# 0411tony/Yue

Hardware: AMD Instinct MI355X
Metric: BPR triplet-updates/sec at k=128 (S-round semantics, user rows sequential; the reference's exact sequential semantics: secondary.exact) (higher is better)
Workload: dtype f32

## Files before the change

yue_amd/csrc/bpr_host.hip:

```cpp
#include "host_common.hpp"

#include "train_kernels.hpp"
#include "round_kernels.hpp"

using yue_host::fail;
using yue_host::kr_of;
static_assert(yue::kNllSlots == yue_host::kNllSlotsHost && yue::kHeaderSlack == yue_host::kHeaderSlackHost, "host_common.hpp mirrors these");

namespace {

yue::TrainArgs make_args(yue_ctx *c, double lr, double regU, double regI) {
    yue::TrainArgs a{};
    a.P = c->P.p; a.Q = c->Q.p; a.dP = c->dP.p; a.dQ = c->dQ.p;
    a.stage = c->Q.p ? c->Q.p + (size_t)c->n * c->k : nullptr;
    a.ev_u = c->ev_u.p; a.ev_i = c->ev_i.p; a.ev_j = c->ev_j.p;
    a.indptr = c->indptr.p; a.indices = c->indices.p;
    a.nll_slots = c->scal.p;
    a.m = c->m; a.n = c->n; a.k = c->k;
    a.lr = lr;
    a.ru = (float)(lr * regU);
    a.ri = (float)(lr * regI);
    a.neg_lo = 0; a.neg_range = (int32_t)c->n;
    return a;
}
// ... 254 lines not shown
            c->Q.release();
            c->Q = bigger;
            a.Q = c->Q.p;
        }
        if (!meta) {
            HIPCHK(c->tab0.resize((size_t)c->n * yue::kStageMax));
            HIPCHK(c->tab1.resize((size_t)c->n * yue::kStageMax));
        }
        a.stage = c->Q.p + (size_t)c->n * c->k;
    }
    std::vector<int64_t> ne;
    for (int64_t r = 0; r < R; ++r) if (bounds[(size_t)r + 1] > bounds[(size_t)r]) ne.push_back(r);
    int rc;
    if (meta) {
        if (!ne.empty() && (rc = launch_round_meta(c, a, bounds))) return rc;
    } else if (!ne.empty()) {
        const int64_t r0 = ne[0];
        if ((rc = launch_round(c, a, 0, 0, bounds[(size_t)r0], bounds[(size_t)r0 + 1], 1, apply_p))) return rc;
    }
    const bool timed = c->timing_stride > 0 && !ne.empty();
    if (timed) {
        if (c->ev_used == c->ev_pool.size()) {
            hipEvent_t s, t;
            HIPCHK(hipEventCreate(&s));
            HIPCHK(hipEventCreate(&t));
            c->ev_pool.emplace_back(s, t);
            c->ev_triplets.push_back(0);
            c->ev_launches.push_back(0);
        }
        HIPCHK(hipEventRecord(c->ev_pool[c->ev_used].first, c->stream));
    }
    size_t pos = 0;
    for (int64_t r = 0; r < R; ++r) {
        if (pos < ne.size() && ne[pos] == r) {
            const int64_t e0 = bounds[(size_t)r], e1 = bounds[(size_t)r + 1];
            int64_t n0 = 0, n1 = 0;
            if (pos + 1 < ne.size()) { n0 = bounds[(size_t)ne[pos + 1]]; n1 = bounds[(size_t)ne[pos + 1] + 1]; }
            const bool seq_user = meta && user_blocks && !c->bigq;
            if ((rc = seq_user ? launch_round_u(c, a, (*user_blocks)[(size_t)r], (*user_blocks)[(size_t)r + 1], e0, e1, r)
                      : meta ? launch_round_m(c, a, e0, e1, r) : launch_round(c, a, e0, e1, n0, n1, (int)(pos & 1), apply_p))) return rc;
            ++pos;
        }
        if ((rc = after_round(r))) return rc;
    }
    if (timed) {
        HIPCHK(hipEventRecord(c->ev_pool[c->ev_used].second, c->stream));
        c->ev_triplets[c->ev_used] = bounds.back() - bounds.front();
        c->ev_launches[c->ev_used] = (int64_t)ne.size();
        c->ev_used++;
    }
    return YUE_OK;
}

void reset_round_state(yue_ctx *c) {
    (void)hipStreamSynchronize(c->stream);
    if (c->cnt0.p) (void)hipMemsetAsync(c->cnt0.p, 0, c->cnt0.n * sizeof(unsigned long long), c->stream);
    if (c->cnt1.p) (void)hipMemsetAsync(c->cnt1.p, 0, c->cnt1.n * sizeof(unsigned long long), c->stream);
    if (c->cntp0.p) (void)hipMemsetAsync(c->cntp0.p, 0, c->cntp0.n * sizeof(uint32_t), c->stream);
    if (c->cntp1.p) (void)hipMemsetAsync(c->cntp1.p, 0, c->cntp1.n * sizeof(uint32_t), c->stream);
    if (c->dP.p) (void)hipMemsetAsync(c->dP.p, 0, c->dP.n * sizeof(float), c->stream);
    if (c->dQ.p) (void)hipMemsetAsync(c->dQ.p, 0, c->dQ.n * sizeof(float), c->stream);
    (void)hipStreamSynchronize(c->stream);
}


}

namespace yue_host {
int zero_scalars(yue_ctx *c) {
    HIPCHK(hipMemsetAsync(c->scal.p, 0, (yue::kNllSlots + 8) * sizeof(double), c->stream));
    return YUE_OK;
}

int read_scalars(yue_ctx *c, double *nll, double *sp, double *sq) {
    double *sc = c->scal.p + yue::kNllSlots;
    hipLaunchKernelGGL(yue::k_sum_slots, dim3(1), dim3(64), 0, c->stream, c->scal.p, yue::kNllSlots, sc);
    double h[3];
    HIPCHK(hipMemcpyAsync(h, sc, sizeof h, hipMemcpyDeviceToHost, c->stream));
    HIPCHK(hipStreamSynchronize(c->stream));
    if (nll) *nll = h[0];
    if (sp) *sp = h[1];
    if (sq) *sq = h[2];
    return YUE_OK;
}

int sumsq_async(yue_ctx *c, const double *p_slots) {
    double *sc = c->scal.p + yue::kNllSlots;
    HIPCHK(hipMemsetAsync(sc + 1, 0, 2 * sizeof(double), c->stream));
    if (p_slots) hipLaunchKernelGGL(yue::k_sum_slots, dim3(1), dim3(64), 0, c->stream, p_slots, yue::kNllSlots, sc + 1);
    else hipLaunchKernelGGL(yue::k_sumsq, dim3(2048), dim3(256), 0, c->stream, c->P.p, c->m * c->k, sc + 1);
    hipLaunchKernelGGL(yue::k_sumsq, dim3(2048), dim3(256), 0, c->stream, c->Q.p, c->n * c->k, sc + 2);
    return YUE_OK;
}

int upload_triplets(yue_ctx *c, const int32_t *u, const int32_t *i, const int32_t *j, int64_t T, bool validate) {
    for (int64_t t = 0; validate && t < T; ++t) {
        if (u[t] < 0 || u[t] >= c->m || i[t] < 0 || i[t] >= c->n || j[t] >= c->n)
            return fail(YUE_ERR_ARG, "triplet " + std::to_string(t) + " out of range");
    }
    HIPCHK(c->xu.resize((size_t)T + yue::kHeaderSlack)); HIPCHK(c->xi.resize((size_t)T + yue::kHeaderSlack)); HIPCHK(c->xj.resize((size_t)T + yue::kHeaderSlack));
    HIPCHK(hipMemcpyAsync(c->xu.p, u, T * sizeof(int32_t), hipMemcpyHostToDevice, c->stream));
    HIPCHK(hipMemcpyAsync(c->xi.p, i, T * sizeof(int32_t), hipMemcpyHostToDevice, c->stream));
    HIPCHK(hipMemcpyAsync(c->xj.p, j, T * sizeof(int32_t), hipMemcpyHostToDevice, c->stream));
    return YUE_OK;
}
}
// ... 106 lines not shown
    }
    HIPCHK(hipGetLastError());
    HIPCHK(hipMemcpyAsync(loss_out, c->x_loss.p, T * sizeof(double), hipMemcpyDeviceToHost, c->stream));
    HIPCHK(hipStreamSynchronize(c->stream));
    return YUE_OK;
}

int yue_adam_reset(yue_ctx *c) {
    if (!c || !c->have_factors) return fail(YUE_ERR_ARG, "yue_adam_reset: no factors uploaded");
    HIPCHK(hipSetDevice(c->device));
    const size_t mk = (size_t)c->m * c->k, nk = (size_t)c->n * c->k;
    HIPCHK(c->aU_m.resize(mk)); HIPCHK(c->aU_v.resize(mk)); HIPCHK(c->aV_m.resize(nk)); HIPCHK(c->aV_v.resize(nk));
    HIPCHK(hipMemsetAsync(c->aU_m.p, 0, mk * sizeof(float), c->stream)); HIPCHK(hipMemsetAsync(c->aU_v.p, 0, mk * sizeof(float), c->stream));
    HIPCHK(hipMemsetAsync(c->aV_m.p, 0, nk * sizeof(float), c->stream)); HIPCHK(hipMemsetAsync(c->aV_v.p, 0, nk * sizeof(float), c->stream));
    HIPCHK(hipMemsetAsync(c->dP.p, 0, mk * sizeof(float), c->stream)); HIPCHK(hipMemsetAsync(c->dQ.p, 0, nk * sizeof(float), c->stream));
    c->adam_m = c->m; c->adam_n = c->n; c->adam_k = c->k;
    return YUE_OK;
}

int yue_adam_step(yue_ctx *c, const int32_t *u, const int32_t *i, const int32_t *j, int64_t T, double lr, double reg, int64_t step, double *loss_out) {
    if (!c || !c->have_factors) return fail(YUE_ERR_ARG, "yue_adam_step: no factors uploaded");
    if (T <= 0 || !u || !i || !j || step < 1) return fail(YUE_ERR_ARG, "yue_adam_step: bad argument (T > 0, step >= 1)");
    HIPCHK(hipSetDevice(c->device));
    if (c->adam_m != c->m || c->adam_n != c->n || c->adam_k != c->k) { const int rc0 = yue_adam_reset(c); if (rc0) return rc0; }
    for (int64_t t = 0; t < T; ++t)
        if (u[t] < 0 || u[t] >= c->m || i[t] < 0 || i[t] >= c->n || j[t] < 0 || j[t] >= c->n) return fail(YUE_ERR_ARG, "yue_adam_step: triplet " + std::to_string(t) + " out of range");
    int rc = upload_triplets(c, u, i, j, T, true);
    if (rc) return rc;
    if ((rc = zero_scalars(c))) return rc;
    yue::MbArgs a{};
    a.U = c->P.p; a.V = c->Q.p; a.gU = c->dP.p; a.gV = c->dQ.p; a.k = c->k; a.u = c->xu.p; a.i = c->xi.p; a.j = c->xj.p; a.T = T;
    a.reg = (float)reg; a.loss_slots = c->scal.p;
    const dim3 grid((unsigned)(((T + 31) / 32 + 3) / 4));
    switch (kr_of(c->k)) {
        case 1: hipLaunchKernelGGL(yue::k_mb_grad<1>, grid, dim3(256), 0, c->stream, a); break;
        case 2: hipLaunchKernelGGL(yue::k_mb_grad<2>, grid, dim3(256), 0, c->stream, a); break;
        default: hipLaunchKernelGGL(yue::k_mb_grad<4>, grid, dim3(256), 0, c->stream, a); break;
    }
    const double b1 = 0.9, b2 = 0.999;
    const float lr_t = (float)(lr * std::sqrt(1.0 - std::pow(b2, (double)step)) / (1.0 - std::pow(b1, (double)step)));
    const int64_t mk = c->m * (int64_t)c->k, nk = c->n * (int64_t)c->k;
    hipLaunchKernelGGL(yue::k_adam, dim3((unsigned)std::min<int64_t>(8192, (mk + 255) / 256)), dim3(256), 0, c->stream, c->P.p, c->aU_m.p, c->aU_v.p, c->dP.p, mk, lr_t, 0.9f, 0.999f, 1e-8f);
    hipLaunchKernelGGL(yue::k_adam, dim3((unsigned)std::min<int64_t>(8192, (nk + 255) / 256)), dim3(256), 0, c->stream, c->Q.p, c->aV_m.p, c->aV_v.p, c->dQ.p, nk, lr_t, 0.9f, 0.999f, 1e-8f);
    HIPCHK(hipGetLastError());
    return read_scalars(c, loss_out, nullptr, nullptr);
}

int yue_sample_negatives(yue_ctx *c, uint64_t seed, uint32_t epoch, int32_t *j_out) {
    if (!c || !c->have_inter || !j_out) return fail(YUE_ERR_ARG, "yue_sample_negatives: no interactions uploaded");
    HIPCHK(hipSetDevice(c->device));
    yue::TrainArgs a = make_args(c, 0, 0, 0);
    a.seed = seed; a.epoch = epoch;
    if (c->E > 0) {
        hipLaunchKernelGGL(yue::k_sample, dim3((unsigned)((c->E + 255) / 256)), dim3(256), 0, c->stream, a, c->E);
        HIPCHK(hipGetLastError());
        HIPCHK(hipMemcpyAsync(j_out, c->ev_j.p, c->E * sizeof(int32_t), hipMemcpyDeviceToHost, c->stream));
    }
    HIPCHK(hipStreamSynchronize(c->stream));
    return YUE_OK;
}

int yue_sumsq(yue_ctx *c, double *sp, double *sq) {
    if (!c || !c->have_factors) return fail(YUE_ERR_ARG, "yue_sumsq: no factors uploaded");
    HIPCHK(hipSetDevice(c->device));
    int rc = sumsq_async(c);
    if (rc) return rc;
    double h[2];
    HIPCHK(hipMemcpyAsync(h, c->scal.p + yue::kNllSlots + 1, sizeof h, hipMemcpyDeviceToHost, c->stream));
    HIPCHK(hipStreamSynchronize(c->stream));
    if (sp) *sp = h[0];
    if (sq) *sq = h[1];
    return YUE_OK;
}

int yue_bpr_epoch(yue_ctx *c, uint64_t seed, uint32_t epoch, int64_t round_events, double lr, double regU, double regI,
                  double *nll_out, double *sumsqP_out, double *sumsqQ_out) {
    if (!c || !c->have_factors || !c->have_inter) return fail(YUE_ERR_ARG, "yue_bpr_epoch: upload factors and interactions first");
    if (round_events < 0) return fail(YUE_ERR_ARG, "yue_bpr_epoch: round_events must be positive (or 0 for the device's default)");
    HIPCHK(hipSetDevice(c->device));
    yue::TrainArgs a = make_args(c, lr, regU, regI);
    a.seed = seed + 0x632BE59BD9B4E019ull * (uint64_t)c->rank;
    a.epoch = epoch;
    int rc = zero_scalars(c);
    if (rc) return rc;
    const int64_t E = c->E;
    if (E > 0) hipLaunchKernelGGL(yue::k_sample, dim3((unsigned)((E + 255) / 256)), dim3(256), 0, c->stream, a, E);
    if (c->opt_epoch_exact) {
        if (yue_host::on_communicator(c) && c->nranks > 1) return fail(YUE_ERR_ARG, "yue_bpr_epoch: option epoch_exact runs on one GPU (the sequential order spans all item shards)");
        if ((rc = yue_host::chain_epoch(c, lr, regU, regI))) return rc;
        if ((rc = sumsq_async(c))) return rc;
        return read_scalars(c, nll_out, sumsqP_out, sumsqQ_out);
    }
    std::vector<int64_t> bounds;
    double tot[2] = {(double)E, (double)c->n};
    if (yue_host::on_communicator(c)) {
        if ((rc = yue_allreduce_f64(c, tot, 2))) return rc;
        if ((rc = zero_scalars(c))) return rc;
    }
    const double etot = tot[0];
    if (round_events == 0 && (rc = default_round_events(c, tot[1] / c->nranks, &round_events))) return rc;
    int64_t ub = 1, group = 1;
    if ((rc = yue_epoch_plan(c->m, c->k, round_events, etot, c->nranks, &ub, &group, nullptr))) return rc;
    if (!yue_host::on_communicator(c)) group = std::max<int64_t>(1, (c->m + ub - 1) / ub);
    else group = std::max<int64_t>(1, ((int64_t)c->opt_comm_group_mb << 20) / std::max<int64_t>(1, ub * c->k * 4));
    std::vector<int64_t> ublock;
    for (int64_t u0 = 0; u0 < c->m; u0 += ub) { ublock.push_back(u0); bounds.push_back(c->h_ev_ptr[(size_t)u0]); }
    ublock.push_back(c->m); bounds.push_back(E);
    const int64_t R = (int64_t)ublock.size() - 1;
    const bool seq_user = !yue_host::on_communicator(c) && c->opt_round_user_seq && meta_path_fits(c);
    if (seq_user) {
        HIPCHK(c->d_ev_ptr.resize((size_t)c->m + 1));
        if (!c->d_ev_ptr_valid) {
            HIPCHK(hipMemcpyAsync(c->d_ev_ptr.p, c->h_ev_ptr.data(), ((size_t)c->m + 1) * sizeof(int64_t), hipMemcpyHostToDevice, c->stream));
            c->d_ev_ptr_valid = true;
        }
        HIPCHK(c->margins.resize((size_t)std::max<int64_t>(E, 1)));
    }
    c->psq_in_rounds = seq_user && c->all_users_have_events && E > 0;
    if (c->psq_in_rounds) {
        HIPCHK(c->psq_slots.resize((size_t)yue::kNllSlots));
        HIPCHK(hipMemsetAsync(c->psq_slots.p, 0, (size_t)yue::kNllSlots * sizeof(double), c->stream));
    }
    c->last_round_user_seq = 0;
    auto after = [&](int64_t r) -> int {
        if (seq_user && !c->bigq) { c->last_round_user_seq = 1; return YUE_OK; }
        if ((r + 1) % group != 0 && r + 1 != R) return YUE_OK;
        const int64_t g_first = ublock[(size_t)(r - (r % group))], g_last = ublock[(size_t)r + 1];
        const int64_t first = g_first * c->k, count = (g_last - g_first) * c->k;
        const dim3 grid((unsigned)std::min<int64_t>(4096, (count + 255) / 256));
        if (!yue_host::on_communicator(c)) {
            hipLaunchKernelGGL(yue::k_apply_range, grid, dim3(256), 0, c->stream, c->P.p, c->dP.p, first, count);
            return YUE_OK;
        }
        HIPCHK(hipEventRecord(c->ev_rounds, c->stream));
        HIPCHK(hipStreamWaitEvent(c->comm_stream, c->ev_rounds, 0));
        c->comm_collectives += 1;
        c->comm_bytes += (double)count * sizeof(float);
        if (const int rcr = yue_host::reduce_user_block(c, first, count, c->comm_stream)) return rcr;
        hipLaunchKernelGGL(yue::k_apply_range, grid, dim3(256), 0, c->comm_stream, c->P.p, c->dP.p, first, count);
        return YUE_OK;
    };
    c->comm_collectives = 0; c->comm_bytes = 0.0; c->comm_wait_ms = 0.0;
    if ((rc = run_rounds(c, a, bounds, 0, after, meta_path_fits(c), seq_user ? &ublock : nullptr))) { reset_round_state(c); return rc; }
    if (c->last_round_user_seq && E > 0)
        hipLaunchKernelGGL(yue::k_loss_margins, dim3(2048), dim3(256), 0, c->stream, c->margins.p, c->ev_j.p, E, c->scal.p);
    const bool psq_done = c->psq_in_rounds && c->last_round_user_seq;
    c->psq_in_rounds = false;
    if (yue_host::on_communicator(c)) {
        HIPCHK(hipEventRecord(c->ev_t_rounds, c->stream));
        HIPCHK(hipEventRecord(c->ev_t_comm, c->comm_stream));
    }
    HIPCHK(hipEventRecord(c->ev_comm, c->comm_stream));
    HIPCHK(hipStreamWaitEvent(c->stream, c->ev_comm, 0));
    c->comm_compute_waits = 1;
    HIPCHK(hipGetLastError());
    if ((rc = sumsq_async(c, psq_done ? c->psq_slots.p : nullptr))) return rc;
    if ((rc = read_scalars(c, nll_out, sumsqP_out, sumsqQ_out))) return rc;
    if (yue_host::on_communicator(c)) {
        float ms = 0.f;
        HIPCHK(hipEventSynchronize(c->ev_t_comm));
        HIPCHK(hipEventElapsedTime(&ms, c->ev_t_rounds, c->ev_t_comm));
        c->comm_wait_ms = ms > 0.f ? ms : 0.0;
    }
    return YUE_OK;
}

int yue_epoch_plan(int64_t m, int k, int64_t round_events, double events_total, int nranks,
                   int64_t *user_block, int64_t *blocks_per_group, int64_t *n_blocks) {
    if (m <= 0 || k <= 0 || round_events <= 0 || nranks < 1 || !(events_total >= 0.0)) return fail(YUE_ERR_ARG, "yue_epoch_plan: bad argument");
    const double per_user = events_total / (double)nranks / (double)m;
    const int64_t ub = std::max<int64_t>(1, (int64_t)std::floor((double)round_events / std::max(per_user, 1e-9) + 0.5));
    if (user_block) *user_block = ub;
    if (blocks_per_group) *blocks_per_group = std::max<int64_t>(1, (8ll << 20) / std::max<int64_t>(1, ub * k * 4));
    if (n_blocks) *n_blocks = (m + ub - 1) / ub;
    return YUE_OK;
}

int yue_default_round_events(yue_ctx *c, int64_t *out) {
    if (!c || !c->have_factors || !out) return fail(YUE_ERR_ARG, "yue_default_round_events: upload factors first (the value depends on k)");
    HIPCHK(hipSetDevice(c->device));
    double n_rows = (double)c->n;
    if (yue_host::on_communicator(c)) {
        const int rc = yue_allreduce_f64(c, &n_rows, 1);
        if (rc) return rc;
        n_rows /= c->nranks;
    }
    return default_round_events(c, n_rows, out);
}

int yue_set_kernel_timing(yue_ctx *c, int stride) {
    if (!c || stride < 0) return fail(YUE_ERR_ARG, "yue_set_kernel_timing: bad argument");
    c->timing_stride = stride;
    c->ev_used = 0;
    return YUE_OK;
}

int yue_get_kernel_timing(yue_ctx *c, double *total_ms, int64_t *launches, int64_t *triplets) {
    if (!c) return fail(YUE_ERR_ARG, "null context");
    HIPCHK(hipSetDevice(c->device));
    HIPCHK(hipStreamSynchronize(c->stream));
    double tot = 0.0;
    int64_t trip = 0, nl = 0;
    for (size_t t = 0; t < c->ev_used; ++t) {
        float ms = 0.f;
        HIPCHK(hipEventElapsedTime(&ms, c->ev_pool[t].first, c->ev_pool[t].second));
        tot += ms;
        trip += c->ev_triplets[t];
        nl += c->ev_launches[t];
    }
    if (total_ms) *total_ms = tot;
// ... 153 lines not shown
```

yue_amd/csrc/round_kernels.hpp:

```cpp
#pragma once
#include "train_kernels.hpp"

#ifdef YUE_ABL_NO_HOT
#define YUE_M_HOT(val, rs, vo, so) asm volatile("" :: "v"(val))
#else
#define YUE_M_HOT(val, rs, vo, so) YUE_BATOMIC(val, rs, vo, so)
#endif
#ifdef YUE_ABL_NO_DP
#define YUE_M_DP(val, rs, vo, so) asm volatile("" :: "v"(val))
#else
#define YUE_M_DP(val, rs, vo, so) YUE_BATOMIC(val, rs, vo, so)
#endif

#define YUE_BLOAD_NT(rs, vo, so) __builtin_bit_cast(float, __builtin_amdgcn_raw_buffer_load_b32((rs), (vo), (so), 2))
#if defined(YUE_EXP_LOAD_CACHED)
#define YUE_M_LOAD_J(rs, vo, so) YUE_BLOAD(rs, vo, so)
#define YUE_M_LOAD_I(rs, vo, so) YUE_BLOAD(rs, vo, so)
#elif defined(YUE_EXP_LOAD_NT)
#define YUE_M_LOAD_J(rs, vo, so) YUE_BLOAD_NT(rs, vo, so)
#define YUE_M_LOAD_I(rs, vo, so) YUE_BLOAD_NT(rs, vo, so)
#else
#define YUE_M_LOAD_J(rs, vo, so) YUE_BLOAD_NT(rs, vo, so)
#define YUE_M_LOAD_I(rs, vo, so) YUE_BLOAD(rs, vo, so)
#endif

#define YUE_FOLD_LD(p) __builtin_nontemporal_load(p)
#define YUE_FOLD_LDROW(p) (*(p))

namespace yue {

constexpr uint32_t kMetaStageMax = 64u;
constexpr uint32_t kMetaStageDefault = 4u;
constexpr uint32_t kMetaUnique = 1u, kMetaStaged = 2u, kMetaHot = 3u;
constexpr uint32_t kMetaFirst = 1u << 31;
constexpr int kMetaUnroll = 8;
__host__ __device__ inline uint32_t meta_kind(uint32_t w) { return w & 3u; }
__host__ __device__ inline uint32_t meta_slot(uint32_t w) { return (w >> 2) & 0x1fffffffu; }
__host__ __device__ inline bool meta_first(uint32_t w) { return (w & kMetaFirst) != 0u; }
__host__ __device__ inline uint32_t fold_count(uint32_t w) { return w >> 25; }
__host__ __device__ inline uint32_t fold_block(uint32_t w) { return w & 0x1ffffffu; }
constexpr uint32_t kLdsStaged = 1u << 31, kLdsTicket = 1u << 25;
static_assert(kMetaStageMax <= 64u, "tickets of a block must fit bits 25..30 of the LDS word");
__device__ inline uint32_t meta_of_staged(uint32_t lds) {
    const uint32_t ticket = (lds >> 25) & 63u;
    return kMetaStaged | (((lds & 0x1ffffffu) + ticket) << 2) | (ticket == 0u ? kMetaFirst : 0u);
}

struct MetaArgs {
    const int32_t *ev_i, *ev_j;
    const int64_t *bounds;
    int64_t R;
    int32_t n;
    int32_t range;
    int32_t G;
    int32_t chunk;
    uint32_t stage_max;
    uint32_t *meta_i, *meta_j;
    unsigned long long *round_rows;
    uint2 *fold;
    const uint2 *bk_touch;
    const uint32_t *bk_ptr;
};

__host__ __device__ inline int64_t fold_base(int64_t e0, int64_t r) { return (e0 + 4 * r + 3) & ~(int64_t)3; }

template <bool BUCKETED>
__global__ void __launch_bounds__(1024) k_round_meta(MetaArgs a) {
    extern __shared__ uint32_t slots[];
    __shared__ unsigned long long wsum[16];
    __shared__ unsigned long long range_base;
    const int tid = threadIdx.x, lane = tid & 63, wv = tid >> 6;
    const int64_t xcd = blockIdx.x & 7, local = blockIdx.x >> 3, per_xcd = gridDim.x >> 3;
    const int64_t rounds_here = (a.R - xcd + 7) >> 3;
    for (int64_t sq = local; sq < rounds_here * a.G; sq += per_xcd) {
        const int64_t r = (sq / a.G) * 8 + xcd;
        const int32_t g = (int32_t)(sq % a.G);
        const int32_t lo = g * a.range;
        const int32_t width = min(a.range, a.n - lo);
        const int64_t e0 = a.bounds[r], e1 = a.bounds[r + 1];
        for (int s = tid; s < a.range; s += 1024) slots[s] = 0u;
        __syncthreads();
        const uint2 *mine_t = nullptr;
        uint32_t mine_n = 0u;
        if (BUCKETED) {
            const uint32_t *bp = a.bk_ptr + r * (a.G + 1) + g;
            mine_t = a.bk_touch + 2 * e0 + bp[0];
            mine_n = bp[1] - bp[0];
        }
        if (BUCKETED) {
            for (uint32_t t = tid; t < mine_n; t += 1024) atomicAdd(&slots[mine_t[t].x - (uint32_t)lo], 1u);
        } else {
        for (int64_t eb = e0 + tid; eb < e1; eb += 1024 * kMetaUnroll) {
            int32_t vi[kMetaUnroll], vj[kMetaUnroll];
#pragma unroll
            for (int q = 0; q < kMetaUnroll; ++q) {
                const int64_t e = eb + 1024 * q;
                vj[q] = e < e1 ? a.ev_j[e] : -1; vi[q] = e < e1 ? a.ev_i[e] : 0;
            }
#pragma unroll
            for (int q = 0; q < kMetaUnroll; ++q)
                if (vj[q] >= 0) {
                    const uint32_t si = (uint32_t)(vi[q] - lo), sj = (uint32_t)(vj[q] - lo);
                    if (si < (uint32_t)width) atomicAdd(&slots[si], 1u);
                    if (sj < (uint32_t)width) atomicAdd(&slots[sj], 1u);
                }
        }
        }
        __syncthreads();
        const int s0 = tid * a.chunk;
        unsigned long long mine = 0ull;
        for (int q = 0; q < a.chunk; ++q) {
            const int s = s0 + q;
            if (s < width) { const uint32_t c = slots[s]; if (c >= 2u) mine += (1ull << 32) + (c <= a.stage_max ? c : 0u); }
        }
        unsigned long long incl = mine;
#pragma unroll
        for (int off = 1; off < 64; off <<= 1) { const unsigned long long up = __shfl_up(incl, off); if (lane >= off) incl += up; }
        if (lane == 63) wsum[wv] = incl;
        __syncthreads();
        if (tid == 0) {
            unsigned long long total = 0ull;
            for (int q = 0; q < 16; ++q) total += wsum[q];
            range_base = total ? atomicAdd(a.round_rows + r, total) : 0ull;
        }
        __syncthreads();
        unsigned long long run = range_base + incl - mine;
        for (int q = 0; q < wv; ++q) run += wsum[q];
        uint2 *fold = a.fold + fold_base(e0, r);
        for (int q = 0; q < a.chunk; ++q) {
            const int s = s0 + q;
            if (s < width) {
                const uint32_t c = slots[s];
                if (c >= 2u) {
                    const bool st = c <= a.stage_max;
                    slots[s] = st ? (kLdsStaged | ((uint32_t)run & 0x1ffffffu)) : kMetaHot;
                    fold[run >> 32] = make_uint2((uint32_t)(lo + s), st ? ((c << 25) | ((uint32_t)run & 0x1ffffffu)) : 0u);
                    run += (1ull << 32) + (st ? c : 0u);
                }
            }
        }
        __syncthreads();
        if (BUCKETED) {
            for (uint32_t t = tid; t < mine_n; t += 1024) {
                const uint2 tc = mine_t[t];
                const uint32_t sl = tc.x - (uint32_t)lo;
                const uint32_t wd = slots[sl];
                const uint32_t mw = (wd & kLdsStaged) ? meta_of_staged(atomicAdd(&slots[sl], kLdsTicket)) : wd;
                ((tc.y & 1u) ? a.meta_j : a.meta_i)[e0 + (tc.y >> 1)] = mw;
            }
        } else
        for (int64_t eb = e0 + tid; eb < e1; eb += 1024 * kMetaUnroll) {
            int32_t vi[kMetaUnroll], vj[kMetaUnroll];
#pragma unroll
            for (int q = 0; q < kMetaUnroll; ++q) {
                const int64_t e = eb + 1024 * q;
                vj[q] = e < e1 ? a.ev_j[e] : -1; vi[q] = e < e1 ? a.ev_i[e] : 0;
            }
#pragma unroll
            for (int q = 0; q < kMetaUnroll; ++q) {
                const int64_t e = eb + 1024 * q;
                if (vj[q] >= 0) {
                    const uint32_t si = (uint32_t)(vi[q] - lo), sj = (uint32_t)(vj[q] - lo);
                    if (si < (uint32_t)width) {
                        const uint32_t wd = slots[si];
                        a.meta_i[e] = (wd & kLdsStaged) ? meta_of_staged(atomicAdd(&slots[si], kLdsTicket)) : wd;
                    }
                    if (sj < (uint32_t)width) {
                        const uint32_t wd = slots[sj];
                        a.meta_j[e] = (wd & kLdsStaged) ? meta_of_staged(atomicAdd(&slots[sj], kLdsTicket)) : wd;
                    }
                } else if (g == 0 && e < e1) {
                    a.meta_i[e] = 0u; a.meta_j[e] = 0u;
                }
            }
        }
        __syncthreads();
    }
}

constexpr int kBucketShift = 15;
constexpr int kBucketRangesMax = 256;
struct BucketArgs {
    const int32_t *ev_i, *ev_j;
    const int64_t *bounds;
    int64_t R;
    int32_t G;
    uint2 *bk_touch;
    uint32_t *bk_ptr;
    uint32_t *meta_i, *meta_j;
};

__global__ void __launch_bounds__(1024) k_round_bucket(BucketArgs a) {
    __shared__ uint32_t cnt[kBucketRangesMax], off[kBucketRangesMax + 1];
    const int tid = threadIdx.x;
    for (int64_t r = blockIdx.x; r < a.R; r += gridDim.x) {
        const int64_t e0 = a.bounds[r], e1 = a.bounds[r + 1];
        for (int g = tid; g < a.G; g += 1024) cnt[g] = 0u;
        __syncthreads();
        for (int64_t eb = e0 + tid; eb < e1; eb += 1024 * kMetaUnroll) {
            int32_t vi[kMetaUnroll], vj[kMetaUnroll];
#pragma unroll
            for (int q = 0; q < kMetaUnroll; ++q) {
                const int64_t e = eb + 1024 * q;
                vj[q] = e < e1 ? a.ev_j[e] : 0; vi[q] = e < e1 ? a.ev_i[e] : -1;
            }
#pragma unroll
            for (int q = 0; q < kMetaUnroll; ++q) {
                if (vi[q] < 0) continue;
                if (vj[q] >= 0) { atomicAdd(&cnt[vi[q] >> kBucketShift], 1u); atomicAdd(&cnt[vj[q] >> kBucketShift], 1u); }
                else { a.meta_i[eb + 1024 * q] = 0u; a.meta_j[eb + 1024 * q] = 0u; }
            }
        }
        __syncthreads();
        if (tid == 0) {
            uint32_t run = 0u;
            for (int g = 0; g < a.G; ++g) { off[g] = run; run += cnt[g]; cnt[g] = 0u; }
            off[a.G] = run;
        }
        __syncthreads();
        for (int g = tid; g <= a.G; g += 1024) a.bk_ptr[r * (a.G + 1) + g] = off[g];
        uint2 *dst = a.bk_touch + 2 * e0;
        for (int64_t eb = e0 + tid; eb < e1; eb += 1024 * kMetaUnroll) {
            int32_t vi[kMetaUnroll], vj[kMetaUnroll];
#pragma unroll
            for (int q = 0; q < kMetaUnroll; ++q) {
                const int64_t e = eb + 1024 * q;
                vj[q] = e < e1 ? a.ev_j[e] : -1; vi[q] = e < e1 ? a.ev_i[e] : 0;
// ... 243 lines not shown
            for (int r = 0; r < KR; ++r) { const float a1 = p[r] * qi[r]; ai = ai + a1; const float a2 = p[r] * qj[r]; aj = aj + a2; }
            const float x = wave_sum(ai) - wave_sum(aj);
            const float c = FAST ? chain_coef_fast(x, lrf) : (float)(a.lr * (1.0 - chain_sigmoid(x)));
            xs = (unsigned)lane == t ? x : xs;
            const unsigned cli = meta_kind(mi), clj = meta_kind(mj);
            const bool uniq_i = cli == kMetaUnique, uniq_j = clj == kMetaUnique;
            const bool full_i = uniq_i || meta_first(mi), full_j = uniq_j || meta_first(mj);
            const unsigned oi = (unsigned)ti * row_bytes, oj = (unsigned)tj * row_bytes;
            const unsigned wi = uniq_i ? oi : stage0 + meta_slot(mi) * row_bytes;
            const unsigned wj = uniq_j ? oj : stage0 + meta_slot(mj) * row_bytes;
            Elem o[KR];
#pragma unroll
            for (int r = 0; r < KR; ++r) { o[r] = bpr_elem(p[r], qi[r], qj[r], c, a.ru, a.ri); p[r] = o[r].p2; }
            if (cli != kMetaHot) {
#pragma unroll
                for (int r = 0; r < KR; ++r) YUE_BSTORE(full_i ? o[r].qi2 : o[r].qi2 - qi[r], rsQ, vo[r], wi);
            } else {
#pragma unroll
                for (int r = 0; r < KR; ++r) YUE_M_HOT(o[r].qi2 - qi[r], rsdQ, vo[r], oi);
            }
            if (clj != kMetaHot) {
#pragma unroll
                for (int r = 0; r < KR; ++r) YUE_BSTORE(full_j ? o[r].qj2 : o[r].qj2 - qj[r], rsQ, vo[r], wj);
            } else {
#pragma unroll
                for (int r = 0; r < KR; ++r) YUE_M_HOT(o[r].qj2 - qj[r], rsdQ, vo[r], oj);
            }
        };
        constexpr int D = KR == 1 ? 8 : 4;
        float qi[D][KR], qj[D][KR];
#pragma unroll
        for (int s_ = 0; s_ < D; ++s_) gather(qi[s_], qj[s_], (unsigned)s_);
        for (unsigned t = 0; t < seg_len; t += D) {
#pragma unroll
            for (int s_ = 0; s_ < D; ++s_) {
                step(qi[s_], qj[s_], t + s_);
                gather(qi[s_], qj[s_], (t + s_ + D) & 63u);
            }
        }
        if ((unsigned)lane < seg_len) ra.margins[e0 + seg + lane] = xs;
    }
#pragma unroll
    for (int r = 0; r < KR; ++r) { const unsigned e = 64u * r + lane; if (e < k) prow[e] = p[r]; }
    if (ra.psq_slots) {
        double s = 0.0;
#pragma unroll
        for (int r = 0; r < KR; ++r) { const unsigned e = 64u * r + lane; const float sq = p[r] * p[r]; if (e < k) s += (double)sq; }
#pragma unroll
        for (int off = 1; off < 64; off <<= 1) s += __shfl_xor(s, off);
        if (lane == 0) atomicAdd(ra.psq_slots + (u & (kNllSlots - 1)), s);
    }
}

__global__ void __launch_bounds__(256) k_loss_margins(const float *__restrict__ x, const int32_t *__restrict__ evj, int64_t E, double *nll_slots) {
    double nl = 0.0;
    const int64_t stride = (int64_t)gridDim.x * blockDim.x;
    for (int64_t e = (int64_t)blockIdx.x * blockDim.x + threadIdx.x; e < E; e += stride)
        if (evj[e] >= 0) nl += -log(chain_sigmoid(x[e]));
#pragma unroll
    for (int off = 1; off < 64; off <<= 1) nl += __shfl_xor(nl, off);
    if ((threadIdx.x & 63) == 0 && nl != 0.0) atomicAdd(nll_slots + ((blockIdx.x * 4 + (threadIdx.x >> 6)) & (kNllSlots - 1)), nl);
}

struct FoldArgs {
    const uint2 *fold;
    const unsigned long long *round_rows;
    float *Q, *dQ;
    const float *stage;
    int k;
    uint32_t capacity;
};

template <int KR, int EPG>
__device__ __forceinline__ void fold_group(const FoldArgs &f, int lane, unsigned k, uint32_t nact, const uint2 (&ent)[4]) {
    float st[EPG][4][KR];
    unsigned el[KR];
    bool big = false;
#pragma unroll
    for (int r = 0; r < KR; ++r) el[r] = min(64u * r + lane, k - 1u);
#pragma unroll
    for (int sl = 0; sl < EPG; ++sl) {
        if ((uint32_t)sl >= nact) continue;
        const uint32_t c = fold_count(ent[sl].y);
        const bool hot = c == 0u;
        const float *src = hot ? f.dQ + (uint64_t)ent[sl].x * k : f.stage + (uint64_t)fold_block(ent[sl].y) * k;
#pragma unroll
        for (int r = 0; r < KR; ++r) st[sl][0][r] = YUE_FOLD_LD(src + el[r]);
        if (hot) {
            const float *row = f.Q + (uint64_t)ent[sl].x * k;
#pragma unroll
            for (int r = 0; r < KR; ++r) st[sl][1][r] = YUE_FOLD_LDROW(row + el[r]);
        } else {
#pragma unroll
            for (int r = 0; r < KR; ++r) st[sl][1][r] = YUE_FOLD_LD(src + (uint64_t)k + el[r]);
        }
        if (c > 2u) {
#pragma unroll
            for (unsigned q = 2; q < 4; ++q)
#pragma unroll
                for (int r = 0; r < KR; ++r) st[sl][q][r] = YUE_FOLD_LD(src + (uint64_t)(q < c ? q : 0u) * k + el[r]);
        }
        big = big || c > 4u;
    }
#pragma unroll
    for (int sl = 0; sl < EPG; ++sl) {
        if ((uint32_t)sl >= nact) continue;
        const uint32_t c = fold_count(ent[sl].y);
        const bool hot = c == 0u;
        float *row = f.Q + (uint64_t)ent[sl].x * k;
        float *dr = f.dQ + (uint64_t)ent[sl].x * k;
#pragma unroll
        for (int r = 0; r < KR; ++r) {
            const unsigned e = 64u * r + lane;
            float acc = st[sl][1][r];
// ... 72 lines not shown
```

yue_amd/csrc/train_kernels.hpp:

```cpp
#pragma once
#include "bpr_device.hpp"

namespace yue {

__global__ void __launch_bounds__(256) k_sample(TrainArgs a, int64_t E) {
    int64_t e = (int64_t)blockIdx.x * blockDim.x + threadIdx.x;
    if (e < E) a.ev_j[e] = sample_negative(a, a.ev_u[e], e);
}

template <int KR>
__global__ void __launch_bounds__(256) k_bpr_level(TrainArgs a, int64_t e_begin, int64_t e_end, int tpw) {
    const int lane = threadIdx.x & 63;
    const int64_t wave = (int64_t)blockIdx.x * (blockDim.x >> 6) + (threadIdx.x >> 6);
    const int64_t base = e_begin + wave * tpw;
    if (base >= e_end) return;
    const int cnt = (int)((e_end - base) < (int64_t)tpw ? (e_end - base) : (int64_t)tpw);
    int u = 0, i = 0, j = 0;
    if (lane < cnt) { u = a.ev_u[base + lane]; i = a.ev_i[base + lane]; j = a.ev_j[base + lane]; }
    const int k = a.k;
    double nll = 0.0;
    for (int t = 0; t < cnt; ++t) {
        const int64_t tu = __builtin_amdgcn_readlane(u, t);
        const int64_t ti = __builtin_amdgcn_readlane(i, t);
        const int64_t tj = __builtin_amdgcn_readlane(j, t);
        float p[KR], qi[KR], qj[KR];
#pragma unroll
        for (int r = 0; r < KR; ++r) {
            const int e = 64 * r + lane;
            p[r] = e < k ? a.P[tu * k + e] : 0.0f;
            qi[r] = e < k ? a.Q[ti * k + e] : 0.0f;
            qj[r] = e < k ? a.Q[tj * k + e] : 0.0f;
        }
        float ai = 0.0f, aj = 0.0f;
#pragma unroll
        for (int r = 0; r < KR; ++r) { const float a1 = p[r] * qi[r]; ai = ai + a1; const float a2 = p[r] * qj[r]; aj = aj + a2; }
        const float x = wave_sum(ai) - wave_sum(aj);
        const double s = 1.0 / (1.0 + exp(-(double)x));
        const float c = (float)(a.lr * (1.0 - s));
        nll += -log(s);
#pragma unroll
        for (int r = 0; r < KR; ++r) {
            const int e = 64 * r + lane;
            const Elem o = bpr_elem(p[r], qi[r], qj[r], c, a.ru, a.ri);
            if (e < k) { a.P[tu * k + e] = o.p2; a.Q[ti * k + e] = o.qi2; a.Q[tj * k + e] = o.qj2; }
        }
    }
    if (lane == 0) atomicAdd(a.nll_slots + (wave & (kNllSlots - 1)), nll);
}

struct MbArgs {
    const float *U, *V;
    float *gU, *gV;
    int k;
    const int32_t *u, *i, *j;
    int64_t T;
    float reg;
    double *loss_slots;
};

template <int KR>
// ... 397 lines not shown
#pragma unroll
                    for (int r = 0; r < KR; ++r) {
                        const unsigned e = 64u * r + lane;
                        if (e < k) { d[sl][r] = atomicExch(dx[sl] + e, 0.0f); x[sl][r] = xp[sl][e]; }
                    }
                }
            }
#pragma unroll
        for (int sl = 0; sl < 4; ++sl)
            if (act[sl]) {
#pragma unroll
                for (int r = 0; r < KR; ++r) {
                    const unsigned e = 64u * r + lane;
                    if (e < k) xp[sl][e] = x[sl][r] + d[sl][r];
                }
            }
    }
    YUE_STAMP(7, "s_waitcnt vmcnt(0)");
#pragma unroll
    for (int off = 1; off < TPW; off <<= 1) nll += __shfl_xor(nll, off);
    if (lane == 0 && nll != 0.0) atomicAdd(a.nll_slots + (wave & (kNllSlots - 1)), nll);
}

__global__ void __launch_bounds__(256) k_apply_range(float *X, float *dX, int64_t first_elem, int64_t count) {
    const int64_t stride = (int64_t)gridDim.x * blockDim.x;
    for (int64_t t = (int64_t)blockIdx.x * blockDim.x + threadIdx.x; t < count; t += stride) {
        const int64_t o = first_elem + t;
        X[o] += dX[o];
        dX[o] = 0.0f;
    }
}

__global__ void __launch_bounds__(256) k_sumsq(const float *X, int64_t count, double *out) {
    __shared__ double part[4];
    double s = 0.0;
    const int64_t stride = (int64_t)gridDim.x * blockDim.x;
    for (int64_t t = (int64_t)blockIdx.x * blockDim.x + threadIdx.x; t < count; t += stride) {
        const float sq = X[t] * X[t];
        s += (double)sq;
    }
    for (int off = 32; off >= 1; off >>= 1) s += __shfl_xor(s, off);
    if ((threadIdx.x & 63) == 0) part[threadIdx.x >> 6] = s;
    __syncthreads();
    if (threadIdx.x == 0) atomicAdd(out, part[0] + part[1] + part[2] + part[3]);
}

__global__ void __launch_bounds__(64) k_sum_slots(const double *slots, int nslots, double *out) {
    double s = 0.0;
    for (int t = threadIdx.x; t < nslots; t += 64) s += slots[t];
    for (int off = 32; off >= 1; off >>= 1) s += __shfl_xor(s, off);
    if (threadIdx.x == 0) *out = s;
}

}
```

Baseline: 1.838 billion.

## Rework negative sampling per user group, vectorize meta scans, fuse epoch reductions

```diff
diff --git a/yue_amd/csrc/bpr_host.hip b/yue_amd/csrc/bpr_host.hip
--- a/yue_amd/csrc/bpr_host.hip
+++ b/yue_amd/csrc/bpr_host.hip
@@ -330,6 +330,22 @@
     return YUE_OK;
 }
 
+int upload_ev_ptr(yue_ctx *c) {
+    HIPCHK(c->d_ev_ptr.resize((size_t)c->m + 1));
+    if (!c->d_ev_ptr_valid) {
+        HIPCHK(hipMemcpyAsync(c->d_ev_ptr.p, c->h_ev_ptr.data(), ((size_t)c->m + 1) * sizeof(int64_t), hipMemcpyHostToDevice, c->stream));
+        c->d_ev_ptr_valid = true;
+    }
+    return YUE_OK;
+}
+
+int launch_sample(yue_ctx *c, const yue::TrainArgs &a) {
+    if (const int rc = upload_ev_ptr(c)) return rc;
+    const int64_t waves = (c->m + yue::kSampleUsers - 1) / yue::kSampleUsers;
+    hipLaunchKernelGGL(yue::k_sample, dim3((unsigned)((waves + 3) / 4)), dim3(256), 0, c->stream, a, c->d_ev_ptr.p);
+    return YUE_OK;
+}
+
 void reset_round_state(yue_ctx *c) {
     (void)hipStreamSynchronize(c->stream);
     if (c->cnt0.p) (void)hipMemsetAsync(c->cnt0.p, 0, c->cnt0.n * sizeof(unsigned long long), c->stream);
@@ -542,7 +558,7 @@
     yue::TrainArgs a = make_args(c, 0, 0, 0);
     a.seed = seed; a.epoch = epoch;
     if (c->E > 0) {
-        hipLaunchKernelGGL(yue::k_sample, dim3((unsigned)((c->E + 255) / 256)), dim3(256), 0, c->stream, a, c->E);
+        if (const int rc = launch_sample(c, a)) return rc;
         HIPCHK(hipGetLastError());
         HIPCHK(hipMemcpyAsync(j_out, c->ev_j.p, c->E * sizeof(int32_t), hipMemcpyDeviceToHost, c->stream));
     }
@@ -574,7 +590,7 @@
     int rc = zero_scalars(c);
     if (rc) return rc;
     const int64_t E = c->E;
-    if (E > 0) hipLaunchKernelGGL(yue::k_sample, dim3((unsigned)((E + 255) / 256)), dim3(256), 0, c->stream, a, E);
+    if (E > 0 && (rc = launch_sample(c, a))) return rc;
     if (c->opt_epoch_exact) {
         if (yue_host::on_communicator(c) && c->nranks > 1) return fail(YUE_ERR_ARG, "yue_bpr_epoch: option epoch_exact runs on one GPU (the sequential order spans all item shards)");
         if ((rc = yue_host::chain_epoch(c, lr, regU, regI))) return rc;
@@ -599,11 +615,7 @@
     const int64_t R = (int64_t)ublock.size() - 1;
     const bool seq_user = !yue_host::on_communicator(c) && c->opt_round_user_seq && meta_path_fits(c);
     if (seq_user) {
-        HIPCHK(c->d_ev_ptr.resize((size_t)c->m + 1));
-        if (!c->d_ev_ptr_valid) {
-            HIPCHK(hipMemcpyAsync(c->d_ev_ptr.p, c->h_ev_ptr.data(), ((size_t)c->m + 1) * sizeof(int64_t), hipMemcpyHostToDevice, c->stream));
-            c->d_ev_ptr_valid = true;
-        }
+        if ((rc = upload_ev_ptr(c))) return rc;
         HIPCHK(c->margins.resize((size_t)std::max<int64_t>(E, 1)));
     }
     c->psq_in_rounds = seq_user && c->all_users_have_events && E > 0;
@@ -632,8 +644,6 @@
     };
     c->comm_collectives = 0; c->comm_bytes = 0.0; c->comm_wait_ms = 0.0;
     if ((rc = run_rounds(c, a, bounds, 0, after, meta_path_fits(c), seq_user ? &ublock : nullptr))) { reset_round_state(c); return rc; }
-    if (c->last_round_user_seq && E > 0)
-        hipLaunchKernelGGL(yue::k_loss_margins, dim3(2048), dim3(256), 0, c->stream, c->margins.p, c->ev_j.p, E, c->scal.p);
     const bool psq_done = c->psq_in_rounds && c->last_round_user_seq;
     c->psq_in_rounds = false;
     if (yue_host::on_communicator(c)) {
@@ -644,8 +654,24 @@
     HIPCHK(hipStreamWaitEvent(c->stream, c->ev_comm, 0));
     c->comm_compute_waits = 1;
     HIPCHK(hipGetLastError());
-    if ((rc = sumsq_async(c, psq_done ? c->psq_slots.p : nullptr))) return rc;
-    if ((rc = read_scalars(c, nll_out, sumsqP_out, sumsqQ_out))) return rc;
+    if (c->last_round_user_seq && E > 0) {
+        double *sc = c->scal.p + yue::kNllSlots;
+        int cus = 0;
+        HIPCHK(hipDeviceGetAttribute(&cus, hipDeviceAttributeMultiprocessorCount, c->device));
+        hipLaunchKernelGGL(yue::k_epoch_sums, dim3((unsigned)(8 * std::max(cus, 1))), dim3(256), 0, c->stream, c->margins.p, c->ev_j.p, E, c->scal.p,
+                           c->Q.p, c->n * (int64_t)c->k, sc + 2);
+        if (!psq_done) hipLaunchKernelGGL(yue::k_sumsq, dim3(2048), dim3(256), 0, c->stream, c->P.p, c->m * c->k, sc + 1);
+        hipLaunchKernelGGL(yue::k_sum_slots2, dim3(2), dim3(64), 0, c->stream, c->scal.p, sc, psq_done ? c->psq_slots.p : nullptr, sc + 1, yue::kNllSlots);
+        double h[3];
+        HIPCHK(hipMemcpyAsync(h, sc, sizeof h, hipMemcpyDeviceToHost, c->stream));
+        HIPCHK(hipStreamSynchronize(c->stream));
+        if (nll_out) *nll_out = h[0];
+        if (sumsqP_out) *sumsqP_out = h[1];
+        if (sumsqQ_out) *sumsqQ_out = h[2];
+    } else {
+        if ((rc = sumsq_async(c, psq_done ? c->psq_slots.p : nullptr))) return rc;
+        if ((rc = read_scalars(c, nll_out, sumsqP_out, sumsqQ_out))) return rc;
+    }
     if (yue_host::on_communicator(c)) {
         float ms = 0.f;
         HIPCHK(hipEventSynchronize(c->ev_t_comm));
diff --git a/yue_amd/csrc/round_kernels.hpp b/yue_amd/csrc/round_kernels.hpp
--- a/yue_amd/csrc/round_kernels.hpp
+++ b/yue_amd/csrc/round_kernels.hpp
@@ -34,6 +34,7 @@
 constexpr uint32_t kMetaUnique = 1u, kMetaStaged = 2u, kMetaHot = 3u;
 constexpr uint32_t kMetaFirst = 1u << 31;
 constexpr int kMetaUnroll = 8;
+constexpr int kMetaVecUnroll = 8;
 __host__ __device__ inline uint32_t meta_kind(uint32_t w) { return w & 3u; }
 __host__ __device__ inline uint32_t meta_slot(uint32_t w) { return (w >> 2) & 0x1fffffffu; }
 __host__ __device__ inline bool meta_first(uint32_t w) { return (w & kMetaFirst) != 0u; }
@@ -64,6 +65,24 @@
 
 __host__ __device__ inline int64_t fold_base(int64_t e0, int64_t r) { return (e0 + 4 * r + 3) & ~(int64_t)3; }
 
+__device__ __forceinline__ void meta_load_events(const MetaArgs &a, int64_t gb, int64_t e0, int64_t e1,
+                                                 int4 (&vi)[kMetaVecUnroll], int4 (&vj)[kMetaVecUnroll]) {
+#pragma unroll
+    for (int q = 0; q < kMetaVecUnroll; ++q) {
+        const int64_t g4 = gb + 4096 * q;
+        if (g4 < e1) {
+            vi[q] = *reinterpret_cast<const int4 *>(a.ev_i + g4); vj[q] = *reinterpret_cast<const int4 *>(a.ev_j + g4);
+        } else { vi[q] = make_int4(0, 0, 0, 0); vj[q] = make_int4(-1, -1, -1, -1); }
+    }
+#pragma unroll
+    for (int q = 0; q < kMetaVecUnroll; ++q)
+#pragma unroll
+        for (int c = 0; c < 4; ++c) {
+            const int64_t e = gb + 4096 * q + c;
+            if (e < e0 || e >= e1) (&vj[q].x)[c] = -1;
+        }
+}
+
 template <bool BUCKETED>
 __global__ void __launch_bounds__(1024) k_round_meta(MetaArgs a) {
     extern __shared__ uint32_t slots[];
@@ -87,22 +106,23 @@
             mine_t = a.bk_touch + 2 * e0 + bp[0];
             mine_n = bp[1] - bp[0];
         }
+        const int64_t ea = e0 & ~(int64_t)3;
         if (BUCKETED) {
             for (uint32_t t = tid; t < mine_n; t += 1024) atomicAdd(&slots[mine_t[t].x - (uint32_t)lo], 1u);
         } else {
-        for (int64_t eb = e0 + tid; eb < e1; eb += 1024 * kMetaUnroll) {
-            int32_t vi[kMetaUnroll], vj[kMetaUnroll];
-#pragma unroll
-            for (int q = 0; q < kMetaUnroll; ++q) {
-                const int64_t e = eb + 1024 * q;
-                vj[q] = e < e1 ? a.ev_j[e] : -1; vi[q] = e < e1 ? a.ev_i[e] : 0;
-            }
-#pragma unroll
-            for (int q = 0; q < kMetaUnroll; ++q)
-                if (vj[q] >= 0) {
-                    const uint32_t si = (uint32_t)(vi[q] - lo), sj = (uint32_t)(vj[q] - lo);
-                    if (si < (uint32_t)width) atomicAdd(&slots[si], 1u);
-                    if (sj < (uint32_t)width) atomicAdd(&slots[sj], 1u);
+        for (int64_t gb = ea + 4 * tid; gb < e1; gb += 4096 * kMetaVecUnroll) {
+            int4 vi[kMetaVecUnroll], vj[kMetaVecUnroll];
+            meta_load_events(a, gb, e0, e1, vi, vj);
+#pragma unroll
+            for (int q = 0; q < kMetaVecUnroll; ++q)
+#pragma unroll
+                for (int c = 0; c < 4; ++c) {
+                    const int32_t ti = (&vi[q].x)[c], tj = (&vj[q].x)[c];
+                    if (tj >= 0) {
+                        const uint32_t si = (uint32_t)(ti - lo), sj = (uint32_t)(tj - lo);
+                        if (si < (uint32_t)width) atomicAdd(&slots[si], 1u);
+                        if (sj < (uint32_t)width) atomicAdd(&slots[sj], 1u);
+                    }
                 }
         }
         }
@@ -149,30 +169,29 @@
                 ((tc.y & 1u) ? a.meta_j : a.meta_i)[e0 + (tc.y >> 1)] = mw;
             }
         } else
-        for (int64_t eb = e0 + tid; eb < e1; eb += 1024 * kMetaUnroll) {
-            int32_t vi[kMetaUnroll], vj[kMetaUnroll];
-#pragma unroll
-            for (int q = 0; q < kMetaUnroll; ++q) {
-                const int64_t e = eb + 1024 * q;
-                vj[q] = e < e1 ? a.ev_j[e] : -1; vi[q] = e < e1 ? a.ev_i[e] : 0;
-            }
-#pragma unroll
-            for (int q = 0; q < kMetaUnroll; ++q) {
-                const int64_t e = eb + 1024 * q;
-                if (vj[q] >= 0) {
-                    const uint32_t si = (uint32_t)(vi[q] - lo), sj = (uint32_t)(vj[q] - lo);
-                    if (si < (uint32_t)width) {
-                        const uint32_t wd = slots[si];
-                        a.meta_i[e] = (wd & kLdsStaged) ? meta_of_staged(atomicAdd(&slots[si], kLdsTicket)) : wd;
+        for (int64_t gb = ea + 4 * tid; gb < e1; gb += 4096 * kMetaVecUnroll) {
+            int4 vi[kMetaVecUnroll], vj[kMetaVecUnroll];
+            meta_load_events(a, gb, e0, e1, vi, vj);
+#pragma unroll
+            for (int q = 0; q < kMetaVecUnroll; ++q)
+#pragma unroll
+                for (int c = 0; c < 4; ++c) {
+                    const int64_t e = gb + 4096 * q + c;
+                    const int32_t ti = (&vi[q].x)[c], tj = (&vj[q].x)[c];
+                    if (tj >= 0) {
+                        const uint32_t si = (uint32_t)(ti - lo), sj = (uint32_t)(tj - lo);
+                        if (si < (uint32_t)width) {
+                            const uint32_t wd = slots[si];
+                            a.meta_i[e] = (wd & kLdsStaged) ? meta_of_staged(atomicAdd(&slots[si], kLdsTicket)) : wd;
+                        }
+                        if (sj < (uint32_t)width) {
+                            const uint32_t wd = slots[sj];
+                            a.meta_j[e] = (wd & kLdsStaged) ? meta_of_staged(atomicAdd(&slots[sj], kLdsTicket)) : wd;
+                        }
+                    } else if (g == 0 && e >= e0 && e < e1) {
+                        a.meta_i[e] = 0u; a.meta_j[e] = 0u;
                     }
-                    if (sj < (uint32_t)width) {
-                        const uint32_t wd = slots[sj];
-                        a.meta_j[e] = (wd & kLdsStaged) ? meta_of_staged(atomicAdd(&slots[sj], kLdsTicket)) : wd;
-                    }
-                } else if (g == 0 && e < e1) {
-                    a.meta_i[e] = 0u; a.meta_j[e] = 0u;
                 }
-            }
         }
         __syncthreads();
     }
@@ -522,14 +541,68 @@
     }
 }
 
-__global__ void __launch_bounds__(256) k_loss_margins(const float *__restrict__ x, const int32_t *__restrict__ evj, int64_t E, double *nll_slots) {
+constexpr float kLossGroupMin = -150.0f;
+constexpr int kLossUnroll = 4;
+__device__ __forceinline__ double loss_of(float x) { return -log(chain_sigmoid(x)); }
+__device__ __forceinline__ double loss_of4(const float4 x, const int4 j) {
+    const float xs[4] = {x.x, x.y, x.z, x.w};
+    const int js[4] = {j.x, j.y, j.z, j.w};
+    const float lowest = fminf(fminf(xs[0], xs[1]), fminf(xs[2], xs[3]));
+    if (!(lowest >= kLossGroupMin) || !(fmaxf(fmaxf(xs[0], xs[1]), fmaxf(xs[2], xs[3])) <= 700.0f)) {
+        double nl = 0.0;
+#pragma unroll
+        for (int c = 0; c < 4; ++c) if (js[c] >= 0) nl += loss_of(xs[c]);
+        return nl;
+    }
+    double prod = 1.0;
+#pragma unroll
+    for (int c = 0; c < 4; ++c) {
+        const double f = 1.0 + chain_exp(-(double)xs[c]);
+        prod = prod * (js[c] >= 0 ? f : 1.0);
+    }
+    return log(prod);
+}
+
+__global__ void __launch_bounds__(256) k_epoch_sums(const float *__restrict__ x, const int32_t *__restrict__ evj, int64_t E, double *nll_slots,
+                                                    const float *__restrict__ Q, int64_t qcount, double *qsq) {
+    __shared__ double part[4];
+    const int64_t tid = (int64_t)blockIdx.x * blockDim.x + threadIdx.x, stride = (int64_t)gridDim.x * blockDim.x;
     double nl = 0.0;
-    const int64_t stride = (int64_t)gridDim.x * blockDim.x;
-    for (int64_t e = (int64_t)blockIdx.x * blockDim.x + threadIdx.x; e < E; e += stride)
-        if (evj[e] >= 0) nl += -log(chain_sigmoid(x[e]));
+    const int64_t E4 = E >> 2;
+    for (int64_t g = tid; g < E4; g += stride * kLossUnroll) {
+        float4 vx[kLossUnroll];
+        int4 vj[kLossUnroll];
+#pragma unroll
+        for (int q = 0; q < kLossUnroll; ++q) {
+            const int64_t gq = g + stride * q;
+            if (gq < E4) { vx[q] = reinterpret_cast<const float4 *>(x)[gq]; vj[q] = reinterpret_cast<const int4 *>(evj)[gq]; }
+            else { vx[q] = make_float4(0.f, 0.f, 0.f, 0.f); vj[q] = make_int4(-1, -1, -1, -1); }
+        }
+#pragma unroll
+        for (int q = 0; q < kLossUnroll; ++q) nl += loss_of4(vx[q], vj[q]);
+    }
+    if (tid == 0) for (int64_t e = E4 << 2; e < E; ++e) if (evj[e] >= 0) nl += loss_of(x[e]);
 #pragma unroll
     for (int off = 1; off < 64; off <<= 1) nl += __shfl_xor(nl, off);
     if ((threadIdx.x & 63) == 0 && nl != 0.0) atomicAdd(nll_slots + ((blockIdx.x * 4 + (threadIdx.x >> 6)) & (kNllSlots - 1)), nl);
+
+    double s = 0.0;
+    const int64_t Q4 = qcount >> 2;
+    for (int64_t g = tid; g < Q4; g += stride * 4) {
+        float4 v[4];
+#pragma unroll
+        for (int q = 0; q < 4; ++q) { const int64_t gq = g + stride * q; v[q] = gq < Q4 ? reinterpret_cast<const float4 *>(Q)[gq] : make_float4(0.f, 0.f, 0.f, 0.f); }
+#pragma unroll
+        for (int q = 0; q < 4; ++q) {
+            const float s0 = v[q].x * v[q].x, s1 = v[q].y * v[q].y, s2 = v[q].z * v[q].z, s3 = v[q].w * v[q].w;
+            s += (double)s0; s += (double)s1; s += (double)s2; s += (double)s3;
+        }
+    }
+    if (tid == 0) for (int64_t t = Q4 << 2; t < qcount; ++t) { const float sq = Q[t] * Q[t]; s += (double)sq; }
+    for (int off = 32; off >= 1; off >>= 1) s += __shfl_xor(s, off);
+    if ((threadIdx.x & 63) == 0) part[threadIdx.x >> 6] = s;
+    __syncthreads();
+    if (threadIdx.x == 0) atomicAdd(qsq, part[0] + part[1] + part[2] + part[3]);
 }
 
 struct FoldArgs {
diff --git a/yue_amd/csrc/train_kernels.hpp b/yue_amd/csrc/train_kernels.hpp
--- a/yue_amd/csrc/train_kernels.hpp
+++ b/yue_amd/csrc/train_kernels.hpp
@@ -3,9 +3,52 @@
 
 namespace yue {
 
-__global__ void __launch_bounds__(256) k_sample(TrainArgs a, int64_t E) {
-    int64_t e = (int64_t)blockIdx.x * blockDim.x + threadIdx.x;
-    if (e < E) a.ev_j[e] = sample_negative(a, a.ev_u[e], e);
+constexpr int kSampleUsers = 8;
+constexpr int kSampleRowWords = 512;
+
+__device__ __forceinline__ int64_t readlane64(int64_t v, int l) {
+    const uint32_t lo = (uint32_t)__builtin_amdgcn_readlane((int)(uint32_t)v, l);
+    const uint32_t hi = (uint32_t)__builtin_amdgcn_readlane((int)(uint32_t)((uint64_t)v >> 32), l);
+    return (int64_t)(((uint64_t)hi << 32) | lo);
+}
+
+__global__ void __launch_bounds__(256) k_sample(TrainArgs a, const int64_t *__restrict__ ev_ptr) {
+    constexpr int G = kSampleUsers;
+    __shared__ int32_t rows_all[4][kSampleRowWords];
+    const int lane = threadIdx.x & 63;
+    const int wv = __builtin_amdgcn_readfirstlane((int)(threadIdx.x >> 6));
+    int32_t *rows = rows_all[wv];
+    const int64_t u0 = ((int64_t)blockIdx.x * 4 + wv) * G;
+    if (u0 >= a.m) return;
+    int64_t ep = 0, ip = 0;
+    if (lane <= G) { const int64_t u = u0 + lane < a.m ? u0 + lane : a.m; ep = ev_ptr[u]; ip = a.indptr[u]; }
+    int64_t eo[G + 1], io[G + 1];
+#pragma unroll
+    for (int q = 0; q <= G; ++q) { eo[q] = readlane64(ep, q); io[q] = readlane64(ip, q); }
+    if (eo[G] <= eo[0]) return;
+    const int64_t span = io[G] - io[0];
+    const int cached = (int)(span < kSampleRowWords ? span : kSampleRowWords);
+    for (int t = lane; t < cached; t += 64) rows[t] = a.indices[io[0] + t];
+    __builtin_amdgcn_wave_barrier();
+    for (int64_t e = eo[0] + lane; e < eo[G]; e += 64) {
+        int64_t lo0 = io[0], hi0 = io[1];
+#pragma unroll
+        for (int q = 1; q < G; ++q) if (e >= eo[q]) { lo0 = io[q]; hi0 = io[q + 1]; }
+        int32_t neg = -1;
+        for (uint32_t t = 0; t < (uint32_t)kMaxAttempts; ++t) {
+            const int32_t c = ctr_draw(a.seed, a.epoch, (uint64_t)e, t, a.neg_lo, a.neg_range);
+            int64_t lo = lo0, hi = hi0;
+            bool found = false;
+            while (lo < hi) {
+                const int64_t mid = (lo + hi) >> 1;
+                const int64_t rel = mid - io[0];
+                const int32_t v = rel < cached ? rows[rel] : a.indices[mid];
+                if (v < c) lo = mid + 1; else if (v > c) hi = mid; else { found = true; break; }
+            }
+            if (!found) { neg = c; break; }
+        }
+        a.ev_j[e] = neg;
+    }
 }
 
 template <int KR>
@@ -509,4 +552,14 @@
     if (threadIdx.x == 0) *out = s;
 }
 
-}
+__global__ void __launch_bounds__(64) k_sum_slots2(const double *slots0, double *out0, const double *slots1, double *out1, int nslots) {
+    const double *slots = blockIdx.x ? slots1 : slots0;
+    double *out = blockIdx.x ? out1 : out0;
+    if (!slots) return;
+    double s = 0.0;
+    for (int t = threadIdx.x; t < nslots; t += 64) s += slots[t];
+    for (int off = 32; off >= 1; off >>= 1) s += __shfl_xor(s, off);
+    if (threadIdx.x == 0) *out = s;
+}
+
+}
```

Measured after the change: 1.861 billion (median of 6 runs). 1.01x the previous value.
